# peterWon/D-LIOM

Measured on AMD Instinct MI355X. Metric: scans/sec (64-beam x 1024 pts -> 10 cm 3D submap), higher is better.
Workload: dtype f32 transforms + u16 voxels/u64 sums (rtcsm), f64 (ceres); 1 GPU; config2 W-dense: 64x1024 scan, all returns matched (adaptive voxel filters neutralised), RTCSM3D + CeresScanMatcher3D(hi+lo) + insertion(hi+lo); N_hi=65536, N_lo=65536, C=35937, linear_window=1, angular_window=5, rescored_candidates_last=2, box_kernel_variant=0, map_scans=20, grids_inserted_into=2, parallelism=replicas x1

## Files before the change

d-liom_amd/csrc/rtcsm3d.hip:

```cpp
#include <algorithm>
#include <chrono>
#include <cmath>
#include <cstdio>
#include <cstdlib>
#include <cstring>
#include <type_traits>
#include <vector>

#include <dlfcn.h>
#include <rccl/rccl.h>

#include "device_common.h"
#include "host_math.h"
#include "probability_values.h"
#include "rtcsm_bounds.h"
#include "rtcsm_candidates.h"
#include "score_box.h"

namespace dliom {

constexpr int kBlock = 256;

template <int PPT, bool WIDE = false>
__global__ __launch_bounds__(kBlock) void rtcsm_score_kernel(
// ... 503 lines not shown
  } else {
    std::vector<char>& host = state_of(ctx)->host_box_tables;
    host.resize(tau_bytes + pass_bytes);
    h = host.data();
  }
  float* const tau = reinterpret_cast<float*>(h);
  Pass* const pass = reinterpret_cast<Pass*>(h + tau_bytes);
  unsigned* const bitmap = reinterpret_cast<unsigned*>(h + tau_bytes + pass_only_bytes + group_bytes);
  std::memset(tau, 0, tau_count * 4);
  std::memset(pass, 0, static_cast<size_t>(passes) * sizeof(Pass));
  double taumax = 0.0;
  for (int tp = 0; tp < passes; ++tp) {
    const int j0 = tp * TC, tc = std::min(TC, T - j0);
    for (int a = 0; a < 3; ++a) {
      double lo = 1e300, hi = -1e300;
      for (int j = j0; j < j0 + tc; ++j) {
        const double v = a == 0 ? c.trans[j].x : (a == 1 ? c.trans[j].y : c.trans[j].z);
        lo = std::min(lo, v);
        hi = std::max(hi, v);
      }
      taumax = std::max(taumax, (hi - lo) * 0.5 / res + 1.0);
    }
  }
  if (rmax + taumax + 130.0 > 1000.0) return (ctx->last_box_refusal = DLIOM_BOX_REFUSED_RANGE, DLIOM_ERR_CAPACITY);
  const double e16 = 1.0 + (2.0 * qmax + rmax + taumax) / 256.0;
  const int B = static_cast<int>(std::ceil(e16 + 0.25));
  const int s_units = B;
  const double u = 1.0 / 65536.0;
  for (int tp = 0; tp < passes; ++tp) {
    Pass& ps = pass[static_cast<size_t>(tp)];
    ps.j0 = tp * TC;
    ps.tc = std::min(TC, T - ps.j0);
    ps.pad[0] = ps.pad[1] = 0;
    for (int a = 0; a < 3; ++a) {
      auto comp = [&](int j) { return static_cast<double>(a == 0 ? c.trans[j].x : (a == 1 ? c.trans[j].y : c.trans[j].z)); };
      double lo = 1e300, hi = -1e300;
      for (int j = ps.j0; j < ps.j0 + ps.tc; ++j) {
        lo = std::min(lo, comp(j));
        hi = std::max(hi, comp(j));
      }
      const double tcen = 0.5 * (lo + hi);
      const double G = tcen / res + 128.5 + s_units * u;
      const double gi = std::floor(G);
      const double f = std::nearbyint((G - gi) * 16384.0) / 16384.0;
      ps.gi[a] = static_cast<int>(gi);
      ps.f[a] = static_cast<float>(f);
      ps.uc[a] = static_cast<float>(tcen / res + 0.5);
      double reach = 0.0;
      for (int jj = 0; jj < TC; ++jj) {
        const int j = ps.j0 + std::min(jj, ps.tc - 1);
        const double tv = comp(j) / res + 128.5 + s_units * u - (gi + f);
        const float tf = static_cast<float>(tv);
        tau[(static_cast<size_t>(tp) * TC + jj) * 4 + a] = tf;
        reach = std::max(reach, std::fabs(static_cast<double>(tf)));
      }
      ps.reach[a] = static_cast<float>(reach + 0.02 + qmax * std::ldexp(1.0, -22));
    }
  }
  std::memset(bitmap, 0, bitmap_count * 4);
  const unsigned thr_units = static_cast<unsigned>(s_units + B);
  for (int tp = 0; tp < passes; ++tp) {
    const Pass& ps = pass[static_cast<size_t>(tp)];
    for (int a = 0; a < 3; ++a) {
      unsigned* words = bitmap + static_cast<size_t>(tp) * kBitmapWords + static_cast<size_t>(a) * (kBuckets / 32);
      for (int jj = 0; jj < ps.tc; ++jj) {
        const double tv = static_cast<double>(tau[(static_cast<size_t>(tp) * TC + jj) * 4 + a]);
        const double af = tv - std::floor(tv);
        const double L = -af - 1.5 * u, H = -af + (thr_units + 1.5) * u;
        const long long b0 = static_cast<long long>(std::floor(L * kBuckets)), b1 = static_cast<long long>(std::floor(H * kBuckets));
        for (long long b = b0; b <= b1; ++b) {
          const unsigned m = static_cast<unsigned>(((b % kBuckets) + kBuckets) % kBuckets);
          words[m >> 5] |= 1u << (m & 31u);
        }
      }
    }
  }
  {
    const double step = c.w.angular_step_size;
    const double a_lanes = (2.0 * c.w.angular_window_size + 1.0) * step;
    const double spread = a_lanes * 0.6 * cloud.max_norm / res;
    const double dim = spread + 2.0 * taumax + 8.0;
    if (dim > kMaxDim || dim * dim * (dim * 0.25) > cells) return (ctx->last_box_refusal = DLIOM_BOX_REFUSED_WINDOW, DLIOM_ERR_CAPACITY);
  }
  if (TC * sizeof(float4) + kBitmapWords * 4 + 16 + static_cast<size_t>(nw) * kListWords * 4 + static_cast<size_t>(cells) * 2 >
      160 * 1024)
    return (ctx->last_box_refusal = DLIOM_BOX_REFUSED_LDS, DLIOM_ERR_CAPACITY);
  struct GroupCache {
    int A = -1, r_first = -1, r_last = -1, nw = 0;
    float step = 0.f;
    std::vector<Group> groups;
  };
  static thread_local GroupCache gcache;
  const bool gcache_hit = gcache.A == c.w.angular_window_size && gcache.step == c.w.angular_step_size &&
                          gcache.r_first == r_first && gcache.r_last == r_last && gcache.nw == nw;
  std::vector<Group>& groups = gcache.groups;
  if (!gcache_hit) {
    gcache.A = -1;
    groups.assign(static_cast<size_t>(rot_blocks), Group());
  }
  for (size_t gi = 0; !gcache_hit && gi < groups.size(); ++gi) {
    Group& gr = groups[gi];
    const int r0 = r_first + static_cast<int>(gi) * nw * 64;
    const int cnt = std::max(0, std::min(nw * 64, r_last - r0));
    gr.c_lane = cnt / 2;
    gr.theta2 = 0.f;
    for (int a = 0; a < 3; ++a) gr.dc[a] = gr.hd[a] = 0.f;
    if (cnt <= 0) {
      gr.c_lane = 0;
      continue;
    }
    RotationSpread sp;
    rotation_spread(c, r0, cnt, &sp);
    const double th = sp.max_angle;
    if (th > 0.3) return (ctx->last_box_refusal = DLIOM_BOX_REFUSED_WINDOW, DLIOM_ERR_CAPACITY);
    for (int a = 0; a < 3; ++a) {
      gr.dc[a] = static_cast<float>(0.5 * (sp.lo[a] + sp.hi[a]));
      gr.hd[a] = static_cast<float>(0.5 * (sp.hi[a] - sp.lo[a]) * 1.0001 + 1e-7);
    }
    gr.theta2 = static_cast<float>(0.51 * th * th * 1.01 + 1e-9);
  }
  gcache.A = c.w.angular_window_size;
  gcache.step = c.w.angular_step_size;
  gcache.r_first = r_first;
  gcache.r_last = r_last;
  gcache.nw = nw;
  DLIOM_PREP_LAP(3);
  struct SpanGuard {
    dliom_ctx* c;
    int span;
    ~SpanGuard() { c->end_span(span); }
  } span_guard{ctx, ctx->begin_span(DLIOM_KERNEL_RTCSM_SCORE)};
  DLIOM_PREP_LAP(4);
  DLIOM_TRY(ctx->box_tables.reserve(tau_bytes + pass_bytes));
  char* base = static_cast<char*>(ctx->box_tables.p);
  const Group* group_src = reinterpret_cast<const Group*>(base + tau_bytes + pass_only_bytes);
  std::memcpy(h + tau_bytes + pass_only_bytes, groups.data(), groups.size() * sizeof(Group));
  if (tables_staged) {
    if (prep_add(prep, base, h, tau_bytes + pass_bytes, 0u))
      group_src = reinterpret_cast<const Group*>(h + tau_bytes + pass_only_bytes);
    else
      DLIOM_HIP_TRY(hipMemcpyAsync(base, h, tau_bytes + pass_bytes, hipMemcpyHostToDevice, ctx->stream));
  } else {
    DLIOM_HIP_TRY(hipMemcpyAsync(base, h, tau_bytes + pass_bytes, hipMemcpyHostToDevice, ctx->stream));
    DLIOM_HIP_TRY(hipStreamSynchronize(ctx->stream));
  }
  Params p;
  p.tau = reinterpret_cast<const float4*>(base);
  p.pass = reinterpret_cast<const Pass*>(base + tau_bytes);
  p.group = reinterpret_cast<const Group*>(base + tau_bytes + pass_only_bytes);
  p.bitmap = reinterpret_cast<const unsigned*>(base + tau_bytes + pass_only_bytes + group_bytes);
  p.trans = d.trans;
  p.rot = d.rot;
  p.sums = d_sums;
  p.error = d_error;
  p.R = R;
  p.r_first = r_first;
  p.r_last = r_last;
  p.T = T;
  p.passes = passes;
  p.n = n;
  p.chunk = std::min(kMaxChunk, std::max(4, chunk_pts & ~3));
  p.order = p.chunk == kCostChunk ? cloud.d_chunk_order : (p.chunk == kCostChunkBig ? cloud.d_chunk_order_big : nullptr);
  p.point_chunks = (n + p.chunk - 1) / p.chunk;
  const int rot_groups = (r_last - r_first + 63) / 64;
  p.rot_groups = rot_groups;
  p.rot_blocks = rot_blocks;
  p.nw = nw;
  p.thr = thr_units;
  p.cells = cells;
  static const int split_points = env_int("DLIOM_BOX_SPLIT", 1);
  p.split_points = split_points;
#ifdef DLIOM_EXPERIMENTS
  static const int box_debug = env_int("DLIOM_BOX_DEBUG", 0);
  p.debug = box_debug;
  if (box_debug & 512) p.order = nullptr;
#else
  p.debug = 0;
#endif
  const size_t lds = TC * sizeof(float4) + kBitmapWords * 4 + 16 + static_cast<size_t>(nw) * kListWords * 4 +
                     static_cast<size_t>(cells) * 2;
  if (lds > 160 * 1024) return (ctx->last_box_refusal = DLIOM_BOX_REFUSED_LDS, DLIOM_ERR_CAPACITY);
  typedef void (*BoxKernel)(GridView, Params, const float*, const float*, const float*);
  const BoxKernel kernel = variant == 0 ? rtcsm_score_box_kernel : (variant == 1 ? rtcsm_score_box_kernel_w3 : rtcsm_score_box_kernel_wide);
  const unsigned attr_bit = variant == 0 ? kFuncAttrScoreBox : (variant == 1 ? kFuncAttrScoreBoxW3 : kFuncAttrScoreBoxWide);
  if ((ctx->func_attr_set & attr_bit) == 0u) {
    DLIOM_HIP_TRY(hipFuncSetAttribute(reinterpret_cast<const void*>(kernel), hipFuncAttributeMaxDynamicSharedMemorySize, 160 * 1024));
    ctx->func_attr_set |= attr_bit;
  }
  ctx->last_box_variant = variant;
  static thread_local size_t resident_lds = 0;
  static thread_local int resident = 0, resident_nw = 0, resident_variant = -1;
  if (resident_lds != lds || resident_nw != nw || resident_variant != variant) {
    resident_nw = nw;
    resident_variant = variant;
    DLIOM_HIP_TRY(hipOccupancyMaxActiveBlocksPerMultiprocessor(&resident, reinterpret_cast<const void*>(kernel), 64 * nw, lds));
    resident_lds = lds;
  }
  const int want_blocks = std::max(1, resident) * ctx->num_cus;
  int slot_quads = std::max(1, want_blocks / std::max(1, rot_blocks * passes));
  slot_quads = std::min(slot_quads, p.point_chunks);
  p.slots = slot_quads;
  p.units = passes * rot_blocks;
  DLIOM_TRY(ctx->box_counters.reserve(static_cast<size_t>(passes) * rot_blocks * 4 + 256));
  if (!prep_add(prep, ctx->box_counters.p, nullptr, static_cast<size_t>(passes) * rot_blocks * 4, 0u))
    DLIOM_HIP_TRY(hipMemsetAsync(ctx->box_counters.p, 0, static_cast<size_t>(passes) * rot_blocks * 4, ctx->stream));
  p.counters = ctx->box_counters.as<unsigned>();
  p.ext_stride = static_cast<int>(cloud.n_padded);
  DLIOM_TRY(ctx->box_extents.reserve(static_cast<size_t>(rot_blocks) * 6 * static_cast<size_t>(cloud.n_padded) * 4));
  p.ext = ctx->box_extents.as<float>();
#ifdef DLIOM_EXPERIMENTS
  g_host_prep.stop();
#endif
  {
    PrepArgs none;
    none.n = 0;
    const PrepArgs& jobs = prep != nullptr ? *prep : none;
    const unsigned prep_rows = jobs.n > 0 ? 1u : 0u;
    hipLaunchKernelGGL(rtcsm_box_extent_kernel, dim3(static_cast<unsigned>((n + 255) / 256), static_cast<unsigned>(rot_blocks) + prep_rows),
                       dim3(256), 0, ctx->stream, p, g.inv_resolution, cloud.d_xs, cloud.d_ys, cloud.d_zs, ctx->box_extents.as<float>(),
                       group_src, d.rot_src, jobs);
    if (prep != nullptr) prep->n = 0;
  }
  const unsigned blocks = static_cast<unsigned>(slot_quads) * passes * rot_blocks;
  hipLaunchKernelGGL(kernel, dim3(blocks), dim3(64 * nw), lds, ctx->stream, g, p, cloud.d_xs, cloud.d_ys, cloud.d_zs);
  DLIOM_HIP_TRY(hipGetLastError());
#ifdef DLIOM_TEST_HOOKS
  if (ctx->tuning[DLIOM_TUNE_RESERVED_TEST_HOOK] == 1) {
    ctx->tuning[DLIOM_TUNE_RESERVED_TEST_HOOK] = 0;
    DLIOM_HIP_TRY(hipMemsetAsync(static_cast<char*>(ctx->box_error.p) + 4, 1, 1, ctx->stream));
  }
#endif
  return DLIOM_OK;
}

constexpr int kScoreTargetBlocks = 8192;

static int launch_score_dense(dliom_ctx* ctx, const dliom_cloud& cloud, const GridView& g, const Candidates& c,
                              const DeviceCandidates& d, int r_first, int r_last, unsigned long long* d_sums,
                              int64_t* processed) {
  const int R = static_cast<int>(c.w.num_rotations), T = static_cast<int>(c.w.num_translations);
  const int n = static_cast<int>(cloud.n);
  const int Rs = r_last - r_first;
  const size_t trans_lds = static_cast<size_t>(T) * 16;
  if (trans_lds > 100 * 1024) return DLIOM_ERR_INVALID_ARGUMENT;
  int bs = kDenseMaxBlock;
  for (int cand = kDenseMaxBlock; cand >= 64; cand -= 64)
    if ((Rs + cand - 1) / cand * cand < (Rs + bs - 1) / bs * bs) bs = cand;
  if (static_cast<int64_t>((Rs + bs - 1) / bs) * ((n + 63) / 64) < 256) bs = 64;
  const int rot_groups = (Rs + bs - 1) / bs;
  int chunk = 4096;
  while (chunk > 8 && static_cast<int64_t>(rot_groups) * ((n + chunk - 1) / chunk) < kScoreTargetBlocks) chunk >>= 1;
  const int point_chunks = (n + chunk - 1) / chunk;
  *processed = static_cast<int64_t>(point_chunks) * chunk;
  DenseDomain dom;
  dom.lo = 0;
  dom.size = g.dense_stride;
  dom.n_real = n;
  dom.pad[0] = dom.pad[1] = dom.pad[2] = kPadCoordinate;
  bool clamp = true;
  {
    float tmax = 0.f, t_init = norm3(c.init.t);
    for (const F3& t : c.trans) tmax = std::max(tmax, std::max(std::fabs(t.x), std::max(std::fabs(t.y), std::fabs(t.z))));
// ... 745 lines not shown
```

d-liom_amd/csrc/score_box.h:

```cpp
#ifndef DLIOM_CSRC_SCORE_BOX_H_
#define DLIOM_CSRC_SCORE_BOX_H_

#include "device_common.h"

namespace dliom {
namespace box {

constexpr int kTC = 27;
#if !defined(DLIOM_EXPERIMENTS) || !defined(DLIOM_BOX_TC_WIDE)
#undef DLIOM_BOX_TC_WIDE
#define DLIOM_BOX_TC_WIDE 49
#endif
constexpr int kTCWide = DLIOM_BOX_TC_WIDE;
#if !defined(DLIOM_EXPERIMENTS) || !defined(DLIOM_BOX_MAX_WAVES)
#undef DLIOM_BOX_MAX_WAVES
#define DLIOM_BOX_MAX_WAVES 4
#endif
constexpr int kWaves = DLIOM_BOX_MAX_WAVES;
constexpr int kMaxDim = 120;
constexpr int kMaxChunk = 64;
constexpr int kBuckets = 8192;
constexpr int kBitmapWords = 3 * kBuckets / 32;
constexpr int kL1Cap = 320;
constexpr int kL2Cap = 128;
#ifndef DLIOM_BOX_HOT_P
#define DLIOM_BOX_HOT_P 4
#endif
constexpr int kHotP = DLIOM_BOX_HOT_P;
#if !defined(DLIOM_EXPERIMENTS) || !defined(DLIOM_BOX_EXP)
#undef DLIOM_BOX_EXP
#define DLIOM_BOX_EXP 0
#endif
#ifdef DLIOM_EXPERIMENTS
#define DLIOM_BOX_DBG(p, bit) (((p).debug & (bit)) != 0)
#define DLIOM_BOX_STAT(p, cond, k, v)                                                                \
  do {                                                                                                \
    if (((p).debug & 128) && (cond)) atomicAdd((p).error + 8 + (k), static_cast<unsigned>(v));        \
  } while (0)
#else
#define DLIOM_BOX_DBG(p, bit) false
#define DLIOM_BOX_STAT(p, cond, k, v) do { } while (0)
#endif
#ifndef DLIOM_BOX_PIPE
#define DLIOM_BOX_PIPE 1
#endif
#ifndef DLIOM_BOX_LATE_ACC
#define DLIOM_BOX_LATE_ACC 1
#endif
constexpr int kPipe = DLIOM_BOX_PIPE;
constexpr bool kLateAcc = DLIOM_BOX_LATE_ACC != 0;
constexpr int kRecords = 8;
constexpr int kListTrash = kL1Cap + kL2Cap + 4 * kRecords;
constexpr int kListWords = kListTrash + 4;

struct Pass {
  int gi[3];
  float f[3];
  float uc[3];
  float reach[3];
  int tc;
  int j0;
  int pad[2];
};

struct Group {
  int c_lane;
  float dc[3];
  float hd[3];
  float theta2;
};

struct Params {
  const float4* tau;
  const Pass* pass;
  const unsigned* bitmap;
  const float* trans;
  const float4* rot;
  const Group* group;
  const float* ext;
  int ext_stride;
  unsigned long long* sums;
  const unsigned* order;
  unsigned* counters;
  unsigned* error;
  int R, r_first, r_last, T, passes;
  int n;
  int chunk;
  int point_chunks, rot_groups, rot_blocks, nw, slots;
  int units;
  unsigned thr;
  int cells;
  int split_points;
  int debug;
};

typedef __attribute__((address_space(3))) const unsigned short lds_cu16;

__device__ __forceinline__ unsigned min_lo16(unsigned running, float w) {
  unsigned r;
  asm("v_min_u32_sdwa %0, %1, %2 dst_sel:DWORD dst_unused:UNUSED_PAD src0_sel:DWORD src1_sel:WORD_0"
      : "=v"(r)
      : "v"(running), "v"(w));
  return r;
}
__device__ __forceinline__ unsigned mad_hi16(float w, unsigned m, unsigned a) {
  unsigned r;
  asm("v_mad_u32_u16 %0, %1, %2, %3 op_sel:[1,0,0,0]" : "=v"(r) : "v"(w), "v"(m), "v"(a));
  return r;
}
typedef float float2v __attribute__((ext_vector_type(2)));
__device__ __forceinline__ float2v pk_add_lo(float2v a, float2v t) {
  float2v r;
  asm("v_pk_add_f32 %0, %1, %2 op_sel_hi:[1,0]" : "=v"(r) : "v"(a), "v"(t));
  return r;
}
__device__ __forceinline__ float2v pk_add_hi(float2v a, float2v t) {
  float2v r;
  asm("v_pk_add_f32 %0, %1, %2 op_sel:[0,1] op_sel_hi:[1,1]" : "=v"(r) : "v"(a), "v"(t));
  return r;
}
__device__ __forceinline__ unsigned to_vgpr(unsigned s) {
  unsigned v;
  asm volatile("v_mov_b32 %0, %1" : "=v"(v) : "s"(s));
  return v;
}
__device__ __forceinline__ float to_vgpr_f(float s) {
  float v;
  asm volatile("v_mov_b32 %0, %1" : "=v"(v) : "s"(s));
  return v;
}
__device__ __forceinline__ float wave_max_f(float v) {
#define DLIOM_DPP_MAX(ctrl, row_mask)                                                                      \
  v = fmaxf(v, __int_as_float(__builtin_amdgcn_update_dpp(__float_as_int(v), __float_as_int(v), ctrl, row_mask, 0xf, false)))
  DLIOM_DPP_MAX(0xB1, 0xf);
  DLIOM_DPP_MAX(0x4E, 0xf);
  DLIOM_DPP_MAX(0x141, 0xf);
  DLIOM_DPP_MAX(0x140, 0xf);
  DLIOM_DPP_MAX(0x142, 0xa);
  DLIOM_DPP_MAX(0x143, 0xc);
#undef DLIOM_DPP_MAX
  return __int_as_float(__builtin_amdgcn_readlane(__float_as_int(v), 63));
}
__device__ __forceinline__ float wave_min_f(float v) { return -wave_max_f(-v); }

struct Geometry {
  int lo[3];
  int dim[3];
  unsigned sx, sxy;
  float kb[3];
};

__device__ __forceinline__ unsigned mirror_value(const GridView& g, int ix, int iy, int iz) {
  const int S = g.dense_stride, B = g.dense_bricks;
  const int mx = ix + g.dense_off[0], my = iy + g.dense_off[1], mz = iz + g.dense_off[2];
  if (mx < 0 || mx >= S || my < 0 || my >= S || mz < 0 || mz >= S) return 1u;
  return g.dense[((static_cast<size_t>(mz >> 2) * B + (my >> 2)) * B + (mx >> 2)) * 64u +
                 static_cast<size_t>(((mz & 3) << 4) | ((my & 3) << 2) | (mx & 3))];
}

struct Lists {
  unsigned* l1;
  unsigned* l2;
  int* rec;
  int n1;
  int seq;
};

__device__ __forceinline__ void resolve_l2(const GridView& g, const Params& p, const Pass& ps, const float4* lds_tau,
                                           const float* __restrict__ px, const float* __restrict__ py,
                                           const float* __restrict__ pz, const Lists& ls, int base1, int n2, int rot0,
                                           int lane) {
  DLIOM_BOX_STAT(p, lane == 0, 6, n2);
  for (int e0 = 0; e0 < n2; e0 += 64) {
    const int e = e0 + lane;
    if (e < n2) {
      const unsigned item = ls.l2[e];
      const unsigned ent = ls.l1[base1 + static_cast<int>(item & 0xFFu)];
      const int j = static_cast<int>(item >> 8);
      const int* rc = ls.rec + 4 * static_cast<int>((ent >> 12) & (kRecords - 1));
      const int r = rot0 + static_cast<int>(ent & 63u), pt = rc[3] + static_cast<int>((ent >> 6) & 63u);
      const float4 qq = p.rot[r];
      const Quat4 q{qq.x, qq.y, qq.z, qq.w};
      float rx, ry, rz;
      rotate_point(q, px[pt], py[pt], pz[pt], rx, ry, rz);
      const float4 t = lds_tau[j];
      const float ax = __builtin_fmaf(rx, g.inv_resolution, static_cast<float>(ps.gi[0] - rc[0]) + ps.f[0]) + t.x;
      const float ay = __builtin_fmaf(ry, g.inv_resolution, static_cast<float>(ps.gi[1] - rc[1]) + ps.f[1]) + t.y;
      const float az = __builtin_fmaf(rz, g.inv_resolution, static_cast<float>(ps.gi[2] - rc[2]) + ps.f[2]) + t.z;
      const int fx = static_cast<int>((__float_as_uint(ax) >> 16) - 0x4300u) + rc[0];
      const int fy = static_cast<int>((__float_as_uint(ay) >> 16) - 0x4300u) + rc[1];
      const int fz = static_cast<int>((__float_as_uint(az) >> 16) - 0x4300u) + rc[2];
      const float* tr = p.trans + 3 * (ps.j0 + j);
      const int ex = cell_of(rx + tr[0], g.resolution), ey = cell_of(ry + tr[1], g.resolution),
                ez = cell_of(rz + tr[2], g.resolution);
      if (ex != fx || ey != fy || ez != fz) {
        if (abs(ex - fx) > 1 || abs(ey - fy) > 1 || abs(ez - fz) > 1) {
          atomicOr(p.error, 1u);
          atomicOr(p.error + 1, 1u);
        }
        const long long delta = static_cast<long long>(mirror_value(g, ex, ey, ez)) -
                                static_cast<long long>(mirror_value(g, fx, fy, fz));
        if (delta != 0)
          atomicAdd(&p.sums[static_cast<size_t>(ps.j0 + j) * p.R + r], static_cast<unsigned long long>(delta));
      }
    }
  }
}

__device__ __forceinline__ void resolve_l1(const GridView& g, const Params& p, const Pass& ps, const float4* lds_tau,
                                           const float* __restrict__ px, const float* __restrict__ py,
                                           const float* __restrict__ pz, const Lists& ls, int base1, int count, int rot0,
                                           int lane) {
  const bool have = lane < count;
  DLIOM_BOX_STAT(p, lane == 0, 4, 1);
  DLIOM_BOX_STAT(p, lane == 0, 5, count);
  float wx = 200.5f, wy = 200.5f, wz = 200.5f;
  if (have) {
    const unsigned ent = ls.l1[base1 + lane];
    const int* rc = ls.rec + 4 * static_cast<int>((ent >> 12) & (kRecords - 1));
    const int r = rot0 + static_cast<int>(ent & 63u), pt = rc[3] + static_cast<int>((ent >> 6) & 63u);
    const float4 qq = p.rot[r];
    const Quat4 q{qq.x, qq.y, qq.z, qq.w};
    float rx, ry, rz;
    rotate_point(q, px[pt], py[pt], pz[pt], rx, ry, rz);
    wx = __builtin_fmaf(rx, g.inv_resolution, static_cast<float>(ps.gi[0] - rc[0]) + ps.f[0]);
    wy = __builtin_fmaf(ry, g.inv_resolution, static_cast<float>(ps.gi[1] - rc[1]) + ps.f[1]);
    wz = __builtin_fmaf(rz, g.inv_resolution, static_cast<float>(ps.gi[2] - rc[2]) + ps.f[2]);
  }
  int n2 = 0;
  for (int j = 0; j < ps.tc; ++j) {
    const float4 t = lds_tau[j];
    unsigned m = min_lo16(0xFFFFFFFFu, wx + t.x);
    m = min_lo16(m, wy + t.y);
// ... 142 lines not shown
      if (false) {
#else
      if (P % 2 == 0) {
#endif
        const float2v txy = {t.x, t.y}, tz0 = {t.z, t.w};
        float2v ax[P / 2 + 1], ay[P / 2 + 1], az[P / 2 + 1];
#pragma unroll
        for (int k = 0; k < P / 2; ++k) {
          ax[k] = pk_add_lo(float2v{wx[2 * k], wx[2 * k + 1]}, txy);
          ay[k] = pk_add_hi(float2v{wy[2 * k], wy[2 * k + 1]}, txy);
          az[k] = pk_add_lo(float2v{wz[2 * k], wz[2 * k + 1]}, tz0);
        }
#pragma unroll
        for (int k = 0; k < P / 2; ++k) {
          a[2 * k] = mad_hi16(ax[k].x, v2, d0);
          a[2 * k + 1] = mad_hi16(ax[k].y, v2, d0);
        }
#pragma unroll
        for (int k = 0; k < P / 2; ++k) {
          a[2 * k] = mad_hi16(ay[k].x, v1, a[2 * k]);
          a[2 * k + 1] = mad_hi16(ay[k].y, v1, a[2 * k + 1]);
        }
#pragma unroll
        for (int k = 0; k < P / 2; ++k) {
          a[2 * k] = mad_hi16(az[k].x, vs2, a[2 * k]);
          a[2 * k + 1] = mad_hi16(az[k].y, vs2, a[2 * k + 1]);
        }
      } else {
#pragma unroll
        for (int k = 0; k < P; ++k) {
          const float ax = wx[k] + t.x, ay = wy[k] + t.y, az = wz[k] + t.z;
          a[k] = mad_hi16(az, vs2, mad_hi16(ay, v1, mad_hi16(ax, v2, d0)));
        }
      }
      if (kLateAcc) __builtin_amdgcn_sched_barrier(0);
      if (j >= kPipe) {
        unsigned s = pv[kPipe - 1][0];
#pragma unroll
        for (int k = 1; k < P; ++k) s += pv[kPipe - 1][k];
        acc[j - kPipe] += s;
        asm volatile("" : "+v"(acc[j - kPipe]));
      }
      if (kLateAcc) __builtin_amdgcn_sched_barrier(0);
      unsigned v[P];
#if DLIOM_BOX_EXP == 1
#pragma unroll
      for (int k = 0; k < P; ++k) v[k] = a[k] & 0x7fffu;
#else
#pragma unroll
      for (int k = 0; k < P; ++k) v[k] = *reinterpret_cast<lds_cu16*>(a[k]);
#endif
#pragma unroll
      for (int d = kPipe - 1; d > 0; --d)
#pragma unroll
        for (int k = 0; k < P; ++k) pv[d][k] = pv[d - 1][k];
#pragma unroll
      for (int k = 0; k < P; ++k) pv[0][k] = v[k];
      t = tn;
      __builtin_amdgcn_sched_barrier(0);
    }
#pragma unroll
    for (int d = kPipe - 1; d >= 0; --d) {
      unsigned s = pv[d][0];
#pragma unroll
      for (int k = 1; k < P; ++k) s += pv[d][k];
      acc[TC - 1 - d] += s;
      asm volatile("" : "+v"(acc[TC - 1 - d]));
    }
  }
  return i;
}

constexpr int kFlushPoints = 131072;
template <int TC>
__device__ __forceinline__ void flush_acc(const Params& p, const Pass& ps, unsigned (&acc)[TC], int r, bool lane_active) {
#pragma unroll
  for (int j = 0; j < TC; ++j) {
    if (lane_active && j < ps.tc && acc[j] != 0u)
      atomicAdd(&p.sums[static_cast<size_t>(ps.j0 + j) * p.R + r], static_cast<unsigned long long>(acc[j]));
    acc[j] = 0u;
  }
}

__device__ __forceinline__ bool box_geometry(const GridView& g, const Params& p, const Pass& ps, const float (&l3)[3],
                                             const float (&h3)[3], int n, int lane, Geometry& geo) {
  const bool have = lane < n;
  bool fits = true;
#pragma unroll
  for (int a = 0; a < 3; ++a) {
    const float l = fmaxf(wave_min_f(have ? l3[a] : 3.0e38f) - ps.reach[a], -1.0e6f);
    const float h = fminf(wave_max_f(have ? h3[a] : -3.0e38f) + ps.reach[a], 1.0e6f);
    geo.lo[a] = __builtin_amdgcn_readfirstlane(static_cast<int>(floorf(l)));
    geo.dim[a] = __builtin_amdgcn_readfirstlane(static_cast<int>(floorf(h))) - geo.lo[a] + 1;
  }
  {
    const int m_lo = (geo.lo[0] + g.dense_off[0]) & ~3;
    const int m_hi = geo.lo[0] + g.dense_off[0] + geo.dim[0];
    geo.lo[0] = m_lo - g.dense_off[0];
    geo.dim[0] = ((m_hi - m_lo) + 3) & ~3;
  }
  geo.sx = static_cast<unsigned>(geo.dim[0]);
  if (((geo.sx >> 2) & 1u) == 0u) geo.sx += 4u;
  const unsigned sy = static_cast<unsigned>(geo.dim[1]) | 1u;
  geo.sxy = geo.sx * sy;
#pragma unroll
  for (int a = 0; a < 3; ++a) {
    fits = fits && geo.dim[a] <= kMaxDim && abs(ps.gi[a] - geo.lo[a]) < 1000;
    geo.kb[a] = static_cast<float>(ps.gi[a] - geo.lo[a]) + ps.f[a];
  }
  fits = fits && static_cast<long long>(geo.sxy) * geo.dim[2] <= p.cells && geo.sxy <= 32767u;
  return fits;
}
__device__ __forceinline__ void point_interval(const Params& p, const Pass& ps, const float* __restrict__ ext_rb, int i,
                                               float (&l3)[3], float (&h3)[3]) {
#pragma unroll
  for (int a = 0; a < 3; ++a) {
    l3[a] = (ext_rb[static_cast<size_t>(2 * a) * p.ext_stride + i] + ps.uc[a]) - 0.0502f;
    h3[a] = (ext_rb[static_cast<size_t>(2 * a + 1) * p.ext_stride + i] + ps.uc[a]) + 0.0502f;
  }
}

__global__ __launch_bounds__(256) void rtcsm_box_extent_kernel(Params p, float inv, const float* __restrict__ px,
                                                               const float* __restrict__ py, const float* __restrict__ pz,
                                                               float* __restrict__ ext, const Group* __restrict__ group_src,
                                                               const float4* __restrict__ rot_src, PrepArgs prep) {
  const int i = blockIdx.x * blockDim.x + threadIdx.x, rb = blockIdx.y;
  if (rb >= p.rot_blocks) {
    prep_block(prep, blockIdx.x, gridDim.x, threadIdx.x, blockDim.x);
    return;
  }
  if (i >= p.n) return;
  const Group grp = group_src[rb];
  const float4 qcc = rot_src[p.r_first + rb * p.nw * 64 + grp.c_lane];
  const Quat4 qc{qcc.x, qcc.y, qcc.z, qcc.w};
  float rabs[9];
  {
    const float w = qc.w, x = qc.x, y = qc.y, z = qc.z;
    rabs[0] = fabsf(1.f - 2.f * (y * y + z * z));
    rabs[1] = fabsf(2.f * (x * y - w * z));
    rabs[2] = fabsf(2.f * (x * z + w * y));
    rabs[3] = fabsf(2.f * (x * y + w * z));
    rabs[4] = fabsf(1.f - 2.f * (x * x + z * z));
    rabs[5] = fabsf(2.f * (y * z - w * x));
    rabs[6] = fabsf(2.f * (x * z - w * y));
    rabs[7] = fabsf(2.f * (y * z + w * x));
    rabs[8] = fabsf(1.f - 2.f * (x * x + y * y));
  }
  const float x = px[i], y = py[i], z = pz[i];
  const float sx_ = grp.dc[1] * z - grp.dc[2] * y, sy_ = grp.dc[2] * x - grp.dc[0] * z, sz_ = grp.dc[0] * y - grp.dc[1] * x;
  float cx, cy, cz;
  rotate_point(qc, x + sx_, y + sy_, z + sz_, cx, cy, cz);
  const float fx = fabsf(x), fy = fabsf(y), fz = fabsf(z);
  const float hx = grp.hd[1] * fz + grp.hd[2] * fy, hy = grp.hd[2] * fx + grp.hd[0] * fz, hz = grp.hd[0] * fy + grp.hd[1] * fx;
  const float m2 = grp.theta2 * (fx + fy + fz) + 1.0e-5f * (fx + fy + fz);
  const float c3[3] = {cx, cy, cz};
  float* out = ext + static_cast<size_t>(rb) * 6 * p.ext_stride + i;
#pragma unroll
  for (int a = 0; a < 3; ++a) {
    const float he = rabs[3 * a] * hx + rabs[3 * a + 1] * hy + rabs[3 * a + 2] * hz + m2;
    out[static_cast<size_t>(2 * a) * p.ext_stride] = (c3[a] - he) * inv;
    out[static_cast<size_t>(2 * a + 1) * p.ext_stride] = (c3[a] + he) * inv;
  }
}

template <int TC>
__device__ __forceinline__ void score_box_body(const GridView& g, const Params& p, const float* __restrict__ px,
                                               const float* __restrict__ py, const float* __restrict__ pz) {
  extern __shared__ float4 lds_dyn4[];
  float4* lds_tau = lds_dyn4;
  unsigned* lds_bitmap = reinterpret_cast<unsigned*>(lds_dyn4 + TC);
  const int wave = __builtin_amdgcn_readfirstlane(static_cast<int>(threadIdx.x >> 6)), lane = threadIdx.x & 63, nthreads = blockDim.x;
  typedef __attribute__((address_space(3))) char lds_char;
  const unsigned lds0 = static_cast<unsigned>(reinterpret_cast<size_t>((lds_char*)lds_dyn4));
  const unsigned tick_off = static_cast<unsigned>(TC * sizeof(float4)) + kBitmapWords * 4u;
  const unsigned lists_off = tick_off + 16u;
  const unsigned box_off = lists_off + static_cast<unsigned>(p.nw) * kListWords * 4u;
  const unsigned box_base = lds0 + box_off;
  unsigned short* box = reinterpret_cast<unsigned short*>(reinterpret_cast<char*>(lds_dyn4) + box_off);
  unsigned* tick = reinterpret_cast<unsigned*>(reinterpret_cast<char*>(lds_dyn4) + tick_off);
  Lists ls;
  ls.l1 = reinterpret_cast<unsigned*>(reinterpret_cast<char*>(lds_dyn4) + lists_off) + wave * kListWords;
  ls.l2 = ls.l1 + kL1Cap;
  ls.rec = reinterpret_cast<int*>(ls.l2 + kL2Cap);
  ls.n1 = 0;
  ls.seq = 0;
  unsigned acc[TC];
#pragma unroll
  for (int j = 0; j < TC; ++j) acc[j] = 0u;
  const int S = g.dense_stride, B = g.dense_bricks;
#ifdef DLIOM_EXPERIMENTS
  unsigned long long stamp_begin = 0ull;
  unsigned stamp_tickets = 0u;
  if (DLIOM_BOX_DBG(p, 256)) stamp_begin = wall_clock64();
#endif
  const int home = static_cast<int>(blockIdx.x % static_cast<unsigned>(p.units));
  const int slot = static_cast<int>(blockIdx.x / static_cast<unsigned>(p.units));
  int parity = 0;
  int loaded_pass = -1;
  const int hops = DLIOM_BOX_DBG(p, 64) ? 1 : p.units;
  for (int hop = 0; hop < hops; ++hop) {
    int unit = home + hop;
    if (unit >= p.units) unit -= p.units;
    unsigned* counter = p.counters + unit;
    int ticket, chunk_id;
    if (hop == 0) {
      ticket = DLIOM_BOX_DBG(p, 8) ? p.point_chunks : slot;
      chunk_id = (p.order != nullptr && ticket < p.point_chunks) ? static_cast<int>(p.order[ticket]) : ticket;
    } else {
      if (threadIdx.x == 0) {
        const int t = p.slots + static_cast<int>(atomicAdd(counter, 1u));
        tick[parity] = static_cast<unsigned>(t);
        tick[2 + parity] = (p.order != nullptr && t < p.point_chunks) ? p.order[t] : static_cast<unsigned>(t);
      }
      __syncthreads();
      ticket = static_cast<int>(tick[parity]);
      chunk_id = static_cast<int>(tick[2 + parity]);
      parity ^= 1;
    }
    if (ticket >= p.point_chunks) continue;
    const int rb = unit % p.rot_blocks;
    const int tp = unit / p.rot_blocks;
    if (tp != loaded_pass) {
      __syncthreads();
      if (threadIdx.x < TC) lds_tau[threadIdx.x] = p.tau[tp * TC + threadIdx.x];
      for (int w = threadIdx.x; w < kBitmapWords; w += nthreads) lds_bitmap[w] = p.bitmap[tp * kBitmapWords + w];
      __syncthreads();
      loaded_pass = tp;
    }
    const int rot_b0 = p.r_first + rb * p.nw * 64;
    const int groups_here = (p.r_last - rot_b0 + 63) >> 6;
    const int split = (p.split_points != 0 && p.nw == 4) ? (groups_here == 1 ? 4 : (groups_here == 2 ? 2 : 1)) : 1;
    const int rot_group = split == 4 ? 0 : (split == 2 ? (wave & 1) : wave);
    const int slice = split == 4 ? wave : (split == 2 ? (wave >> 1) : 0);
    const int rot0 = rot_b0 + rot_group * 64;
    const bool wave_active = rot0 < p.r_last && slice < split;
    const Pass ps = p.pass[tp];
    const bool lane_active = rot0 + lane < p.r_last;
    const float4 qq = p.rot[lane_active ? rot0 + lane : (wave_active ? rot0 : rot_b0)];
    const Quat4 q{qq.x, qq.y, qq.z, qq.w};
    const float* ext_rb = p.ext + static_cast<size_t>(rb) * 6 * p.ext_stride;
    int n_guess = p.chunk;
    int since_flush = 0;
    while (ticket < p.point_chunks) {
      unsigned next_raw = 0u, next_chunk = 0u;
      bool drawn = false;
#ifdef DLIOM_EXPERIMENTS
      ++stamp_tickets;
#endif
      {
        const int c = __builtin_amdgcn_readfirstlane(chunk_id);
        const int c_begin = c * p.chunk, c_end = min(c_begin + p.chunk, p.n);
        int lo = c_begin;
        while (lo < c_end) {
          int n;
          Geometry geo;
          bool fits_out = false;
          {
            n = min(c_end - lo, n_guess);
            float l3[3], h3[3];
            point_interval(p, ps, ext_rb, lo + (lane < n ? lane : 0), l3, h3);
            for (;;) {
              fits_out = box_geometry(g, p, ps, l3, h3, n, lane, geo);
              DLIOM_BOX_STAT(p, threadIdx.x == 0, 7, 1);
              if (fits_out) break;
              if (n == 1) break;
              n = n > 4 ? (((n >> 1) + 3) & ~3) : (n >> 1);
            }
          }
          n_guess = min(p.chunk, n >= 4 ? 2 * n : 4);
          if (since_flush + n > kFlushPoints) {
            flush_acc(p, ps, acc, rot0 + lane, lane_active);
            since_flush = 0;
          }
          since_flush += fits_out ? n : 1;
          if (!fits_out) {
            if (slice == 0) {
              float rx, ry, rz;
              rotate_point(q, px[lo], py[lo], pz[lo], rx, ry, rz);
#pragma unroll
              for (int j = 0; j < TC; ++j) {
                const float* tr = p.trans + 3 * (ps.j0 + min(j, ps.tc - 1));
                acc[j] += mirror_value(g, cell_of(rx + tr[0], g.resolution), cell_of(ry + tr[1], g.resolution),
                                       cell_of(rz + tr[2], g.resolution));
              }
            }
            lo += 1;
            DLIOM_BOX_STAT(p, threadIdx.x == 0, 3, 1);
            continue;
          }
          if (!drawn && (lo + n >= c_end || DLIOM_BOX_DBG(p, 1024))) {
            if (threadIdx.x == 0) next_raw = atomicAdd(counter, 1u);
            drawn = true;
          }
          DLIOM_BOX_STAT(p, threadIdx.x == 0, 0, 1);
          DLIOM_BOX_STAT(p, threadIdx.x == 0, 1, (geo.dim[0] >> 2) * geo.dim[1] * geo.dim[2]);
          DLIOM_BOX_STAT(p, threadIdx.x == 0, 2, n);
          __syncthreads();
          if (!DLIOM_BOX_DBG(p, 2)) {
            const unsigned quads = static_cast<unsigned>(geo.dim[0]) >> 2, dim1 = static_cast<unsigned>(geo.dim[1]);
            const unsigned total = __umul24(__umul24(quads, dim1), static_cast<unsigned>(geo.dim[2]));
            const float inv_q = 1.0f / static_cast<float>(quads), inv_dy = 1.0f / static_cast<float>(dim1);
            const int bx0 = geo.lo[0] + g.dense_off[0], by0 = geo.lo[1] + g.dense_off[1], bz0 = geo.lo[2] + g.dense_off[2];
            const unsigned uB = static_cast<unsigned>(B), uBB = __umul24(uB, uB), uS = static_cast<unsigned>(S);
            const char* dense_bytes = reinterpret_cast<const char*>(g.dense);
#pragma unroll 4
            for (unsigned e = threadIdx.x; e < total; e += static_cast<unsigned>(nthreads)) {
              const unsigned row = static_cast<unsigned>((static_cast<float>(e) + 0.5f) * inv_q);
              const unsigned xq = e - __umul24(row, quads);
              const unsigned z = static_cast<unsigned>((static_cast<float>(row) + 0.5f) * inv_dy);
              const unsigned y = row - __umul24(z, dim1);
              const int mx = bx0 + static_cast<int>(4u * xq), my = by0 + static_cast<int>(y), mz = bz0 + static_cast<int>(z);
              unsigned long long val = 0x0001000100010001ull;
              if (static_cast<unsigned>(mx) < 4u * uB && static_cast<unsigned>(my) < uS && static_cast<unsigned>(mz) < uS) {
                const unsigned umx = static_cast<unsigned>(mx), umy = static_cast<unsigned>(my), umz = static_cast<unsigned>(mz);
                const unsigned off = ((__umul24(umz >> 2, uBB) + __umul24(umy >> 2, uB) + (umx >> 2)) << 7) |
                                     (((umz & 3u) << 5) | ((umy & 3u) << 3));
                val = *reinterpret_cast<const unsigned long long*>(dense_bytes + off);
              }
              *reinterpret_cast<unsigned long long*>(box + (__umul24(z, geo.sxy) + __umul24(y, geo.sx) + 4u * xq)) = val;
            }
          }
          const unsigned rec_id = static_cast<unsigned>(ls.seq & (kRecords - 1));
          if (lane < 4) ls.rec[4 * rec_id + lane] = lane < 3 ? geo.lo[lane] : lo;
          ++ls.seq;
          __syncthreads();
          if (drawn && threadIdx.x == 0) {
            const int t = p.slots + static_cast<int>(next_raw);
            next_chunk = (p.order != nullptr && t < p.point_chunks) ? p.order[t] : static_cast<unsigned>(t);
          }
          if (wave_active && !DLIOM_BOX_DBG(p, 4)) {
            const int part = split > 1 ? ((((n + split - 1) >> (split == 4 ? 2 : 1)) + 3) & ~3) : n;
            const int s_lo = lo + min(n, slice * part), s_n = min(n, (slice + 1) * part) - min(n, slice * part);
            int i = s_lo;
            const int e8 = kHotP == 8 ? s_lo + (s_n & ~7) : s_lo, e4 = s_lo + (s_n & ~3), e1 = s_lo + s_n;
            for (;;) {
              if (kHotP == 8 && i < e8)
                i = main_loop<kHotP, TC>(g, p, geo, q, px, py, pz, i, e8, lo, lds_tau, lds_bitmap, box_base, ls, rec_id, lane_active, lane, acc);
              if (i >= e8 && i < e4)
                i = main_loop<4, TC>(g, p, geo, q, px, py, pz, i, e4, lo, lds_tau, lds_bitmap, box_base, ls, rec_id, lane_active, lane, acc);
              if (i >= e4 && i < e1)
                i = main_loop<1, TC>(g, p, geo, q, px, py, pz, i, e1, lo, lds_tau, lds_bitmap, box_base, ls, rec_id, lane_active, lane, acc);
              if (i >= e1) break;
              drain_l1(g, p, ps, lds_tau, px, py, pz, ls, false, rot0, lane);
            }
            if (!DLIOM_BOX_DBG(p, 1) && (ls.n1 >= 64 || (ls.seq & (kRecords - 1)) == 0))
              drain_l1(g, p, ps, lds_tau, px, py, pz, ls, (ls.seq & (kRecords - 1)) == 0, rot0, lane);
          }
          lo += n;
        }
      }
      if (threadIdx.x == 0) {
        if (!drawn) {
          const int t = p.slots + static_cast<int>(atomicAdd(counter, 1u));
          next_raw = static_cast<unsigned>(t - p.slots);
          next_chunk = (p.order != nullptr && t < p.point_chunks) ? p.order[t] : static_cast<unsigned>(t);
        }
        tick[parity] = static_cast<unsigned>(p.slots) + next_raw;
        tick[2 + parity] = next_chunk;
      }
      __syncthreads();
      ticket = static_cast<int>(tick[parity]);
      chunk_id = static_cast<int>(tick[2 + parity]);
      parity ^= 1;
    }
    if (wave_active && !DLIOM_BOX_DBG(p, 1)) drain_l1(g, p, ps, lds_tau, px, py, pz, ls, true, rot0, lane);
    ls.n1 = 0;
    if (DLIOM_BOX_DBG(p, 16)) {
#pragma unroll
      for (int j = 0; j < TC; ++j) {
        if (lane_active && j < ps.tc)
          atomicAdd(&p.sums[static_cast<size_t>(ps.j0 + j) * p.R + rot0 + lane], static_cast<unsigned long long>(acc[j]));
        acc[j] = 0u;
      }
    } else if (!DLIOM_BOX_DBG(p, 32)) {
      flush_acc(p, ps, acc, rot0 + lane, lane_active);
    }
  }
#ifdef DLIOM_EXPERIMENTS
  if (DLIOM_BOX_DBG(p, 256) && threadIdx.x == 0 && blockIdx.x < 4096u) {
    unsigned long long* st = reinterpret_cast<unsigned long long*>(p.error + 64) + 4 * blockIdx.x;
    unsigned xcc;
    asm volatile("s_getreg_b32 %0, hwreg(HW_REG_XCC_ID)" : "=s"(xcc));
    st[0] = stamp_begin;
    st[1] = wall_clock64();
    st[2] = stamp_tickets;
    st[3] = xcc;
  }
#endif
}


__global__ __launch_bounds__(64 * kWaves) __attribute__((amdgpu_waves_per_eu(4, 8))) void rtcsm_score_box_kernel(
    GridView g, Params p, const float* __restrict__ px, const float* __restrict__ py, const float* __restrict__ pz) {
  score_box_body<kTC>(g, p, px, py, pz);
}
__global__ __launch_bounds__(64 * kWaves) __attribute__((amdgpu_waves_per_eu(3, 8))) void rtcsm_score_box_kernel_w3(
    GridView g, Params p, const float* __restrict__ px, const float* __restrict__ py, const float* __restrict__ pz) {
  score_box_body<kTC>(g, p, px, py, pz);
}
__global__ __launch_bounds__(64 * kWaves) __attribute__((amdgpu_waves_per_eu(3, 8))) void rtcsm_score_box_kernel_wide(
    GridView g, Params p, const float* __restrict__ px, const float* __restrict__ py, const float* __restrict__ pz) {
  score_box_body<kTCWide>(g, p, px, py, pz);
// ... 7 lines not shown
```

Measured before the change: 1049 scans/s.

## Plan box size in one wave via prefix scans and batch box fill loads

Box geometry is now planned once by wave 0 with DPP prefix min/max scans and a ballot over all candidate prefix sizes, replacing the iterative halving loop that redid full wave reductions each attempt. The plan is written to double-buffered LDS slots and read back uniformly by all waves after the existing barrier. The box fill loop is restructured to issue four unconditional (clamped) global loads before the LDS stores, increasing memory-level parallelism. Branch hints and asm barriers are added around rare flush and fallback paths, and the LDS tick region grows slightly.

```diff
diff --git a/d-liom_amd/csrc/box_plan.h b/d-liom_amd/csrc/box_plan.h
--- /dev/null
+++ b/d-liom_amd/csrc/box_plan.h
@@ -0,0 +1,110 @@
+#ifndef DLIOM_CSRC_BOX_PLAN_H_
+#define DLIOM_CSRC_BOX_PLAN_H_
+
+#include <math.h>
+
+#if defined(__HIPCC__) || defined(__CUDACC__)
+#define DLIOM_PLAN_FN __host__ __device__ __forceinline__
+#define DLIOM_PLAN_UNROLL _Pragma("unroll")
+#else
+#define DLIOM_PLAN_FN inline
+#define DLIOM_PLAN_UNROLL
+#endif
+
+namespace dliom {
+namespace box {
+
+constexpr int kMaxDim = 120;
+constexpr int kMaxChunk = 64;
+
+struct Pass {
+  int gi[3];
+  float f[3];
+  float uc[3];
+  float reach[3];
+  int tc;
+  int j0;
+  int pad[2];
+};
+
+struct Geometry {
+  int lo[3];
+  int dim[3];
+  unsigned sx, sxy;
+  float kb[3];
+};
+
+DLIOM_PLAN_FN bool prefix_geometry(const float (&l3)[3], const float (&h3)[3], const Pass& ps, const int (&dense_off)[3],
+                                   int cells, int max_dim, Geometry& geo) {
+  DLIOM_PLAN_UNROLL
+  for (int a = 0; a < 3; ++a) {
+    const float l = fmaxf(l3[a] - ps.reach[a], -1.0e6f);
+    const float h = fminf(h3[a] + ps.reach[a], 1.0e6f);
+    geo.lo[a] = static_cast<int>(floorf(l));
+    geo.dim[a] = static_cast<int>(floorf(h)) - geo.lo[a] + 1;
+  }
+  {
+    const int m_lo = (geo.lo[0] + dense_off[0]) & ~3;
+    const int m_hi = geo.lo[0] + dense_off[0] + geo.dim[0];
+    geo.lo[0] = m_lo - dense_off[0];
+    geo.dim[0] = ((m_hi - m_lo) + 3) & ~3;
+  }
+  geo.sx = static_cast<unsigned>(geo.dim[0]);
+  if (((geo.sx >> 2) & 1u) == 0u) geo.sx += 4u;
+  const unsigned sy = static_cast<unsigned>(geo.dim[1]) | 1u;
+  geo.sxy = geo.sx * sy;
+  bool fits = true;
+  DLIOM_PLAN_UNROLL
+  for (int a = 0; a < 3; ++a) {
+    const int d = ps.gi[a] - geo.lo[a];
+    fits = fits && geo.dim[a] <= max_dim && (d < 0 ? -d : d) < 1000;
+    geo.kb[a] = static_cast<float>(d) + ps.f[a];
+  }
+  return fits && static_cast<long long>(geo.sxy) * geo.dim[2] <= cells && geo.sxy <= 32767u;
+}
+
+DLIOM_PLAN_FN int plan_size(unsigned long long fit_mask, int n_first, bool* fits, int* attempts) {
+  int n = n_first, tried = 1;
+  for (;;) {
+    if ((fit_mask >> (n - 1)) & 1ull) {
+      *fits = true;
+      break;
+    }
+    if (n == 1) {
+      *fits = false;
+      break;
+    }
+    n = n > 4 ? (((n >> 1) + 3) & ~3) : (n >> 1);
+    ++tried;
+  }
+  *attempts = tried;
+  return n;
+}
+
+struct Plan {
+  int n;
+  bool fits;
+  int attempts;
+  Geometry geo;
+};
+
+DLIOM_PLAN_FN Plan plan_box(const float (&lmin)[3][kMaxChunk], const float (&hmax)[3][kMaxChunk], const Pass& ps,
+                            const int (&dense_off)[3], int cells, int max_dim, int n_first) {
+  unsigned long long mask = 0ull;
+  for (int k = 0; k < n_first; ++k) {
+    const float l3[3] = {lmin[0][k], lmin[1][k], lmin[2][k]}, h3[3] = {hmax[0][k], hmax[1][k], hmax[2][k]};
+    Geometry geo;
+    if (prefix_geometry(l3, h3, ps, dense_off, cells, max_dim, geo)) mask |= 1ull << k;
+  }
+  Plan pl;
+  pl.n = plan_size(mask, n_first, &pl.fits, &pl.attempts);
+  const int k = pl.n - 1;
+  const float l3[3] = {lmin[0][k], lmin[1][k], lmin[2][k]}, h3[3] = {hmax[0][k], hmax[1][k], hmax[2][k]};
+  prefix_geometry(l3, h3, ps, dense_off, cells, max_dim, pl.geo);
+  return pl;
+}
+
+}
+}
+
+#endif
diff --git a/d-liom_amd/csrc/rtcsm3d.hip b/d-liom_amd/csrc/rtcsm3d.hip
--- a/d-liom_amd/csrc/rtcsm3d.hip
+++ b/d-liom_amd/csrc/rtcsm3d.hip
@@ -609,7 +609,7 @@
     const double dim = spread + 2.0 * taumax + 8.0;
     if (dim > kMaxDim || dim * dim * (dim * 0.25) > cells) return (ctx->last_box_refusal = DLIOM_BOX_REFUSED_WINDOW, DLIOM_ERR_CAPACITY);
   }
-  if (TC * sizeof(float4) + kBitmapWords * 4 + 16 + static_cast<size_t>(nw) * kListWords * 4 + static_cast<size_t>(cells) * 2 >
+  if (TC * sizeof(float4) + kBitmapWords * 4 + kTickBytes + static_cast<size_t>(nw) * kListWords * 4 + static_cast<size_t>(cells) * 2 >
       160 * 1024)
     return (ctx->last_box_refusal = DLIOM_BOX_REFUSED_LDS, DLIOM_ERR_CAPACITY);
   struct GroupCache {
@@ -704,7 +704,7 @@
 #else
   p.debug = 0;
 #endif
-  const size_t lds = TC * sizeof(float4) + kBitmapWords * 4 + 16 + static_cast<size_t>(nw) * kListWords * 4 +
+  const size_t lds = TC * sizeof(float4) + kBitmapWords * 4 + kTickBytes + static_cast<size_t>(nw) * kListWords * 4 +
                      static_cast<size_t>(cells) * 2;
   if (lds > 160 * 1024) return (ctx->last_box_refusal = DLIOM_BOX_REFUSED_LDS, DLIOM_ERR_CAPACITY);
   typedef void (*BoxKernel)(GridView, Params, const float*, const float*, const float*);
diff --git a/d-liom_amd/csrc/score_box.h b/d-liom_amd/csrc/score_box.h
--- a/d-liom_amd/csrc/score_box.h
+++ b/d-liom_amd/csrc/score_box.h
@@ -1,6 +1,7 @@
 #ifndef DLIOM_CSRC_SCORE_BOX_H_
 #define DLIOM_CSRC_SCORE_BOX_H_
 
+#include "box_plan.h"
 #include "device_common.h"
 
 namespace dliom {
@@ -17,8 +18,6 @@
 #define DLIOM_BOX_MAX_WAVES 4
 #endif
 constexpr int kWaves = DLIOM_BOX_MAX_WAVES;
-constexpr int kMaxDim = 120;
-constexpr int kMaxChunk = 64;
 constexpr int kBuckets = 8192;
 constexpr int kBitmapWords = 3 * kBuckets / 32;
 constexpr int kL1Cap = 320;
@@ -52,16 +51,6 @@
 constexpr int kRecords = 8;
 constexpr int kListTrash = kL1Cap + kL2Cap + 4 * kRecords;
 constexpr int kListWords = kListTrash + 4;
-
-struct Pass {
-  int gi[3];
-  float f[3];
-  float uc[3];
-  float reach[3];
-  int tc;
-  int j0;
-  int pad[2];
-};
 
 struct Group {
   int c_lane;
@@ -129,26 +118,19 @@
   asm volatile("v_mov_b32 %0, %1" : "=v"(v) : "s"(s));
   return v;
 }
-__device__ __forceinline__ float wave_max_f(float v) {
+__device__ __forceinline__ float wave_prefix_max_f(float v) {
 #define DLIOM_DPP_MAX(ctrl, row_mask)                                                                      \
   v = fmaxf(v, __int_as_float(__builtin_amdgcn_update_dpp(__float_as_int(v), __float_as_int(v), ctrl, row_mask, 0xf, false)))
-  DLIOM_DPP_MAX(0xB1, 0xf);
-  DLIOM_DPP_MAX(0x4E, 0xf);
-  DLIOM_DPP_MAX(0x141, 0xf);
-  DLIOM_DPP_MAX(0x140, 0xf);
+  DLIOM_DPP_MAX(0x111, 0xf);
+  DLIOM_DPP_MAX(0x112, 0xf);
+  DLIOM_DPP_MAX(0x114, 0xf);
+  DLIOM_DPP_MAX(0x118, 0xf);
   DLIOM_DPP_MAX(0x142, 0xa);
   DLIOM_DPP_MAX(0x143, 0xc);
 #undef DLIOM_DPP_MAX
-  return __int_as_float(__builtin_amdgcn_readlane(__float_as_int(v), 63));
-}
-__device__ __forceinline__ float wave_min_f(float v) { return -wave_max_f(-v); }
-
-struct Geometry {
-  int lo[3];
-  int dim[3];
-  unsigned sx, sxy;
-  float kb[3];
-};
+  return v;
+}
+__device__ __forceinline__ float wave_prefix_min_f(float v) { return -wave_prefix_max_f(-v); }
 
 __device__ __forceinline__ unsigned mirror_value(const GridView& g, int ix, int iy, int iz) {
   const int S = g.dense_stride, B = g.dense_bricks;
@@ -457,35 +439,9 @@
   }
 }
 
-__device__ __forceinline__ bool box_geometry(const GridView& g, const Params& p, const Pass& ps, const float (&l3)[3],
-                                             const float (&h3)[3], int n, int lane, Geometry& geo) {
-  const bool have = lane < n;
-  bool fits = true;
-#pragma unroll
-  for (int a = 0; a < 3; ++a) {
-    const float l = fmaxf(wave_min_f(have ? l3[a] : 3.0e38f) - ps.reach[a], -1.0e6f);
-    const float h = fminf(wave_max_f(have ? h3[a] : -3.0e38f) + ps.reach[a], 1.0e6f);
-    geo.lo[a] = __builtin_amdgcn_readfirstlane(static_cast<int>(floorf(l)));
-    geo.dim[a] = __builtin_amdgcn_readfirstlane(static_cast<int>(floorf(h))) - geo.lo[a] + 1;
-  }
-  {
-    const int m_lo = (geo.lo[0] + g.dense_off[0]) & ~3;
-    const int m_hi = geo.lo[0] + g.dense_off[0] + geo.dim[0];
-    geo.lo[0] = m_lo - g.dense_off[0];
-    geo.dim[0] = ((m_hi - m_lo) + 3) & ~3;
-  }
-  geo.sx = static_cast<unsigned>(geo.dim[0]);
-  if (((geo.sx >> 2) & 1u) == 0u) geo.sx += 4u;
-  const unsigned sy = static_cast<unsigned>(geo.dim[1]) | 1u;
-  geo.sxy = geo.sx * sy;
-#pragma unroll
-  for (int a = 0; a < 3; ++a) {
-    fits = fits && geo.dim[a] <= kMaxDim && abs(ps.gi[a] - geo.lo[a]) < 1000;
-    geo.kb[a] = static_cast<float>(ps.gi[a] - geo.lo[a]) + ps.f[a];
-  }
-  fits = fits && static_cast<long long>(geo.sxy) * geo.dim[2] <= p.cells && geo.sxy <= 32767u;
-  return fits;
-}
+constexpr int kPlanWords = 12;
+constexpr unsigned kTickBytes = 16u + 2u * kPlanWords * 4u;
+
 __device__ __forceinline__ void point_interval(const Params& p, const Pass& ps, const float* __restrict__ ext_rb, int i,
                                                float (&l3)[3], float (&h3)[3]) {
 #pragma unroll
@@ -493,6 +449,63 @@
     l3[a] = (ext_rb[static_cast<size_t>(2 * a) * p.ext_stride + i] + ps.uc[a]) - 0.0502f;
     h3[a] = (ext_rb[static_cast<size_t>(2 * a + 1) * p.ext_stride + i] + ps.uc[a]) + 0.0502f;
   }
+}
+
+__device__ __forceinline__ void plan_box_wave(const GridView& g, const Params& p, const Pass& ps,
+                                              const float* __restrict__ ext_rb, int first, int n_first, int lane,
+                                              unsigned* plan) {
+  float l3[3], h3[3];
+  point_interval(p, ps, ext_rb, first + (lane < n_first ? lane : 0), l3, h3);
+#pragma unroll
+  for (int a = 0; a < 3; ++a) {
+    l3[a] = wave_prefix_min_f(l3[a]);
+    h3[a] = wave_prefix_max_f(h3[a]);
+  }
+  unsigned long long mask;
+  {
+    Geometry mine;
+    mask = __builtin_amdgcn_ballot_w64(prefix_geometry(l3, h3, ps, g.dense_off, p.cells, kMaxDim, mine));
+  }
+  bool fits;
+  int attempts;
+  const int n = plan_size(mask, n_first, &fits, &attempts);
+  DLIOM_BOX_STAT(p, lane == 0, 7, attempts);
+  float lu[3], hu[3];
+#pragma unroll
+  for (int a = 0; a < 3; ++a) {
+    lu[a] = __int_as_float(__builtin_amdgcn_readlane(__float_as_int(l3[a]), n - 1));
+    hu[a] = __int_as_float(__builtin_amdgcn_readlane(__float_as_int(h3[a]), n - 1));
+  }
+  Geometry geo;
+  prefix_geometry(lu, hu, ps, g.dense_off, p.cells, kMaxDim, geo);
+  if (lane == 0) {
+    uint4* out = reinterpret_cast<uint4*>(plan);
+    out[0] = make_uint4(static_cast<unsigned>(n) | (fits ? 256u : 0u), static_cast<unsigned>(geo.lo[0]),
+                        static_cast<unsigned>(geo.lo[1]), static_cast<unsigned>(geo.lo[2]));
+    out[1] = make_uint4(static_cast<unsigned>(geo.dim[0]), static_cast<unsigned>(geo.dim[1]),
+                        static_cast<unsigned>(geo.dim[2]), geo.sx);
+    out[2].x = geo.sxy;
+  }
+}
+__device__ __forceinline__ int read_plan(const unsigned* plan, const Pass& ps, bool& fits, Geometry& geo) {
+  const uint4* in = reinterpret_cast<const uint4*>(plan);
+  const uint4 a = in[0], b = in[1];
+  const unsigned c = in[2].x;
+#define DLIOM_UNI(x) static_cast<unsigned>(__builtin_amdgcn_readfirstlane(static_cast<int>(x)))
+  const unsigned head = DLIOM_UNI(a.x);
+  geo.lo[0] = static_cast<int>(DLIOM_UNI(a.y));
+  geo.lo[1] = static_cast<int>(DLIOM_UNI(a.z));
+  geo.lo[2] = static_cast<int>(DLIOM_UNI(a.w));
+  geo.dim[0] = static_cast<int>(DLIOM_UNI(b.x));
+  geo.dim[1] = static_cast<int>(DLIOM_UNI(b.y));
+  geo.dim[2] = static_cast<int>(DLIOM_UNI(b.z));
+  geo.sx = DLIOM_UNI(b.w);
+  geo.sxy = DLIOM_UNI(c);
+#undef DLIOM_UNI
+#pragma unroll
+  for (int k = 0; k < 3; ++k) geo.kb[k] = static_cast<float>(ps.gi[k] - geo.lo[k]) + ps.f[k];
+  fits = (head & 256u) != 0u;
+  return static_cast<int>(head & 255u);
 }
 
 __global__ __launch_bounds__(256) void rtcsm_box_extent_kernel(Params p, float inv, const float* __restrict__ px,
@@ -548,7 +561,7 @@
   typedef __attribute__((address_space(3))) char lds_char;
   const unsigned lds0 = static_cast<unsigned>(reinterpret_cast<size_t>((lds_char*)lds_dyn4));
   const unsigned tick_off = static_cast<unsigned>(TC * sizeof(float4)) + kBitmapWords * 4u;
-  const unsigned lists_off = tick_off + 16u;
+  const unsigned lists_off = tick_off + kTickBytes;
   const unsigned box_off = lists_off + static_cast<unsigned>(p.nw) * kListWords * 4u;
   const unsigned box_base = lds0 + box_off;
   unsigned short* box = reinterpret_cast<unsigned short*>(reinterpret_cast<char*>(lds_dyn4) + box_off);
@@ -571,6 +584,8 @@
   const int home = static_cast<int>(blockIdx.x % static_cast<unsigned>(p.units));
   const int slot = static_cast<int>(blockIdx.x / static_cast<unsigned>(p.units));
   int parity = 0;
+  unsigned* plans = tick + 4;
+  int plan_set = 0;
   int loaded_pass = -1;
   const int hops = DLIOM_BOX_DBG(p, 64) ? 1 : p.units;
   for (int hop = 0; hop < hops; ++hop) {
@@ -627,34 +642,30 @@
         const int c_begin = c * p.chunk, c_end = min(c_begin + p.chunk, p.n);
         int lo = c_begin;
         while (lo < c_end) {
-          int n;
+          unsigned* plan = plans + plan_set * kPlanWords;
+          if (wave == 0) plan_box_wave(g, p, ps, ext_rb, lo, min(c_end - lo, n_guess), lane, plan);
+          plan_set ^= 1;
+          __syncthreads();
           Geometry geo;
-          bool fits_out = false;
-          {
-            n = min(c_end - lo, n_guess);
-            float l3[3], h3[3];
-            point_interval(p, ps, ext_rb, lo + (lane < n ? lane : 0), l3, h3);
-            for (;;) {
-              fits_out = box_geometry(g, p, ps, l3, h3, n, lane, geo);
-              DLIOM_BOX_STAT(p, threadIdx.x == 0, 7, 1);
-              if (fits_out) break;
-              if (n == 1) break;
-              n = n > 4 ? (((n >> 1) + 3) & ~3) : (n >> 1);
-            }
-          }
+          bool fits_out;
+          const int n = read_plan(plan, ps, fits_out, geo);
           n_guess = min(p.chunk, n >= 4 ? 2 * n : 4);
-          if (since_flush + n > kFlushPoints) {
-            flush_acc(p, ps, acc, rot0 + lane, lane_active);
+          if (__builtin_expect(since_flush + n > kFlushPoints, 0)) {
+            int r_mine = rot0 + lane;
+            asm volatile("" : "+v"(r_mine));
+            flush_acc(p, ps, acc, r_mine, lane_active);
             since_flush = 0;
           }
           since_flush += fits_out ? n : 1;
-          if (!fits_out) {
+          if (__builtin_expect(!fits_out, 0)) {
             if (slice == 0) {
               float rx, ry, rz;
               rotate_point(q, px[lo], py[lo], pz[lo], rx, ry, rz);
+              int j_first = ps.j0;
+              asm volatile("" : "+s"(j_first));
 #pragma unroll
               for (int j = 0; j < TC; ++j) {
-                const float* tr = p.trans + 3 * (ps.j0 + min(j, ps.tc - 1));
+                const float* tr = p.trans + 3 * (j_first + min(j, ps.tc - 1));
                 acc[j] += mirror_value(g, cell_of(rx + tr[0], g.resolution), cell_of(ry + tr[1], g.resolution),
                                        cell_of(rz + tr[2], g.resolution));
               }
@@ -670,7 +681,6 @@
           DLIOM_BOX_STAT(p, threadIdx.x == 0, 0, 1);
           DLIOM_BOX_STAT(p, threadIdx.x == 0, 1, (geo.dim[0] >> 2) * geo.dim[1] * geo.dim[2]);
           DLIOM_BOX_STAT(p, threadIdx.x == 0, 2, n);
-          __syncthreads();
           if (!DLIOM_BOX_DBG(p, 2)) {
             const unsigned quads = static_cast<unsigned>(geo.dim[0]) >> 2, dim1 = static_cast<unsigned>(geo.dim[1]);
             const unsigned total = __umul24(__umul24(quads, dim1), static_cast<unsigned>(geo.dim[2]));
@@ -678,21 +688,30 @@
             const int bx0 = geo.lo[0] + g.dense_off[0], by0 = geo.lo[1] + g.dense_off[1], bz0 = geo.lo[2] + g.dense_off[2];
             const unsigned uB = static_cast<unsigned>(B), uBB = __umul24(uB, uB), uS = static_cast<unsigned>(S);
             const char* dense_bytes = reinterpret_cast<const char*>(g.dense);
-#pragma unroll 4
-            for (unsigned e = threadIdx.x; e < total; e += static_cast<unsigned>(nthreads)) {
-              const unsigned row = static_cast<unsigned>((static_cast<float>(e) + 0.5f) * inv_q);
-              const unsigned xq = e - __umul24(row, quads);
-              const unsigned z = static_cast<unsigned>((static_cast<float>(row) + 0.5f) * inv_dy);
-              const unsigned y = row - __umul24(z, dim1);
-              const int mx = bx0 + static_cast<int>(4u * xq), my = by0 + static_cast<int>(y), mz = bz0 + static_cast<int>(z);
-              unsigned long long val = 0x0001000100010001ull;
-              if (static_cast<unsigned>(mx) < 4u * uB && static_cast<unsigned>(my) < uS && static_cast<unsigned>(mz) < uS) {
+            const unsigned step = static_cast<unsigned>(nthreads);
+            for (unsigned e0 = threadIdx.x; e0 < total; e0 += 4u * step) {
+              unsigned long long val[4];
+              unsigned dst[4];
+              bool inside[4];
+#pragma unroll
+              for (int k = 0; k < 4; ++k) {
+                const unsigned e = min(e0 + static_cast<unsigned>(k) * step, total - 1u);
+                const unsigned row = static_cast<unsigned>((static_cast<float>(e) + 0.5f) * inv_q);
+                const unsigned xq = e - __umul24(row, quads);
+                const unsigned z = static_cast<unsigned>((static_cast<float>(row) + 0.5f) * inv_dy);
+                const unsigned y = row - __umul24(z, dim1);
+                const int mx = bx0 + static_cast<int>(4u * xq), my = by0 + static_cast<int>(y), mz = bz0 + static_cast<int>(z);
+                inside[k] = static_cast<unsigned>(mx) < 4u * uB && static_cast<unsigned>(my) < uS && static_cast<unsigned>(mz) < uS;
                 const unsigned umx = static_cast<unsigned>(mx), umy = static_cast<unsigned>(my), umz = static_cast<unsigned>(mz);
                 const unsigned off = ((__umul24(umz >> 2, uBB) + __umul24(umy >> 2, uB) + (umx >> 2)) << 7) |
                                      (((umz & 3u) << 5) | ((umy & 3u) << 3));
-                val = *reinterpret_cast<const unsigned long long*>(dense_bytes + off);
+                val[k] = *reinterpret_cast<const unsigned long long*>(dense_bytes + (inside[k] ? off : 0u));
+                dst[k] = __umul24(z, geo.sxy) + __umul24(y, geo.sx) + 4u * xq;
               }
-              *reinterpret_cast<unsigned long long*>(box + (__umul24(z, geo.sxy) + __umul24(y, geo.sx) + 4u * xq)) = val;
+#pragma unroll
+              for (int k = 0; k < 4; ++k)
+                if (e0 + static_cast<unsigned>(k) * step < total)
+                  *reinterpret_cast<unsigned long long*>(box + dst[k]) = inside[k] ? val[k] : 0x0001000100010001ull;
             }
           }
           const unsigned rec_id = static_cast<unsigned>(ls.seq & (kRecords - 1));
```

Measured after the change: 1062 scans/s, median of 6. About the same (+1.2%).
